# wsakobe/CylinderTag

Measured on AMD Instinct MI355X. Metric: frames/sec detect() 1920x1080, higher is better.
Workload: dtype u8; 1 GPU; synthetic 1920x1080 random-stripe frames, 4096 per step over 1 GPU(s), 4 planted CTag_2f12c markers each, detect(img,5,true,5), inputs resident in HBM; frames_per_gpu=4096, chunk=4096, parallelism=frames sharded, dp1, gather=none (1 GPU)

## Files before the change

### cylindertag_amd/csrc/ctag_internal.h

```cpp
#pragma once
#include <hip/hip_runtime.h>
#include <stddef.h>
#include <stdint.h>

#include <vector>

#include "../../include/ctag_types.h"

struct ctag_handle;
struct ctag_camera;
struct ctag_pose_rec;
struct ctag_rig_pose_rec;
struct ctag_mv_pose_rec;
struct ctag_camera_set;

namespace ctag {
template <class T>
struct DevBuf {
    T* p = nullptr;
    size_t cap = 0;
    DevBuf() = default;
    DevBuf(const DevBuf&) = delete;
    DevBuf& operator=(const DevBuf&) = delete;
    ~DevBuf() { release(); }
// ... 282 lines not shown
    CclForm ccl;
    bool latency;
    bool small_cfg;
    bool refprm;
    bool mask_scan, prescan;
    bool all_wave, fork;
    int pack_max, big_points, pack_gx, scan_gx, mscan_gx, big_cols, big_max_gx, welsch_gs, welsch_gx;
    RefineForm refine; int refine_gx, refine_sums_gx;
    bool ccl_stamps, quad_stamps, feat_stamps;
};
ChunkPlan plan_chunk(const PlanIn& in);

hipError_t launch_zero_counters(const ChunkPlan& pl, const Workspace& ws, hipStream_t s);
hipError_t launch_decimate(const ChunkPlan& pl, const uint8_t* frames, ptrdiff_t frame_stride, ptrdiff_t row_stride, const Workspace& ws, hipStream_t s);
hipError_t launch_threshold_ccl(const ChunkPlan& pl, const Workspace& ws, hipStream_t s);
hipError_t launch_seam_merge(const ChunkPlan& pl, const Workspace& ws, hipStream_t s);
hipError_t launch_resolve(const ChunkPlan& pl, const Workspace& ws, hipStream_t s);
hipError_t launch_candidates(const ChunkPlan& pl, const Workspace& ws, hipStream_t s);
hipError_t launch_quads(const ChunkPlan& pl, const Workspace& ws, hipStream_t s, hipEvent_t* ev5 = nullptr);
hipError_t launch_line_fits(const ChunkPlan& pl, const Workspace& ws, hipStream_t s, unsigned long long* stamps = nullptr, hipEvent_t ev_sorted = nullptr);
int welsch_limits(int32_t* out, int capacity);
hipError_t launch_features(const ChunkPlan& pl, const Workspace& ws, const DetectParams& p, hipStream_t s);
hipError_t launch_edge_refine(const ChunkPlan& pl, const uint8_t* frames, ptrdiff_t frame_stride, ptrdiff_t row_stride, const Workspace& ws, const DetectParams& p, hipStream_t s);
hipError_t launch_markers(const ChunkPlan& pl, const Workspace& ws, const DetectParams& p, ctag_frame_result* out, const PendingCtx& pend, hipStream_t s);
hipError_t launch_counters(int nframes, const Workspace& ws, const ctag_frame_result* results, long long* out10, hipStream_t s);
size_t threshold_ccl_lds_bytes(int tw);
bool build_threshold_table(float dark_cap, uint8_t* table , int* dim, int* tcap);
void build_pick_table(uint8_t* table, uint16_t* table16);


enum SiblingState { kPoseState, kDrawState, kRigState, kGatherState, kMvState, kCovState, kFitState, kRigFitState, kCamFitState, kIntrFitState, kRobustState, kTrackState, kHandEyeState, kNumSiblingStates };
void** handle_state_slot(struct ::ctag_handle* h, SiblingState which, void (*free_fn)(void*));
int model_to_device(struct ::ctag_model* m, int device);
int rigs_to_device(struct ::ctag_rigs* r, int device);
bool camera_ok(const struct ::ctag_camera* c);
bool handle_timing(const struct ::ctag_handle* h);
int handle_finish_pending(struct ::ctag_handle* h);
bool handle_pending_state(struct ::ctag_handle* h, const int32_t** count_dev, uint64_t* gen);
void handle_pending_clean(struct ::ctag_handle* h, uint64_t gen);
int handle_device(const struct ::ctag_handle* h);
int handle_dict_cols(const struct ::ctag_handle* h);

struct HandleView {
    int device;
    const Workspace* ws;
    int last_chunk_frames;
// ... 39 lines not shown
```

### cylindertag_amd/csrc/k_feature.hip

```cpp
#include "ctag_internal.h"
#include "ctag_math.h"
#include "ctag_refine.h"
#include "ctag_wave.h"

namespace ctag {

constexpr double kPi = 3.1415926535897932384626433832795;

struct P2 {
    float x, y;
};
__device__ __forceinline__ float dist2p(P2 a, P2 b) { return ctm::sqrt32((a.x - b.x) * (a.x - b.x) + (a.y - b.y) * (a.y - b.y)); }
__device__ __forceinline__ double angdeg(float dy, float dx) { return ctm::atan2_32(dy, dx) * 180 / kPi; }

struct QuadDerived {
    float cx, cy, d[4], a1, a2;
    float e[4];
};
static_assert(sizeof(QuadDerived) == 48, "workspace carve in ctag_api.hip");
struct FeatPtrs {
    const int32_t* ncand;
    const QuadOut* quads;
    QuadDerived* derived;
    int32_t* quad_index;
// ... 433 lines not shown
    const double* Ll = A + ((it + 1) & 3) * 12 + 6;
    const double A00 = Ln[3], A01 = -Ll[3];
    const double A10 = -Ln[2], A11 = Ll[2];
    const double B0 = -Ln[0] + Ll[0];
    const double B1 = -Ln[1] + Ll[1];
    const double det = A00 * A11 - A10 * A01;
    const double W00 = A11 / det, W01 = -A01 / det;
    const double L0 = W00 * B0 + W01 * B1;
    const int idx = ((it + 1) & 3) + off;
    if (ctm::fabs64(det) > 0.001) {
        O->c[2 * idx] = (float)(Ln[0] + L0 * A00);
        O->c[2 * idx + 1] = (float)(Ln[1] + L0 * A10);
    } else {
        O->c[2 * idx] = F->c[2 * idx];
        O->c[2 * idx + 1] = F->c[2 * idx + 1];
    }
}

#if defined(CTAG_REFINE_PLAIN_SYNC) && CTAG_REFINE_PLAIN_SYNC
__device__ __forceinline__ void refine_sync() { __syncthreads(); }
__device__ __forceinline__ void sums_sync() { __syncthreads(); }
#else
__device__ __forceinline__ void refine_sync() { lds_barrier(); }
__device__ __forceinline__ void sums_sync() { lds_wait(); }
#endif
template <int MODE, int REGION = kRefineRegion>
__device__ __forceinline__ bool refine_quad(const RefinePtrs& P, int rows, int cols, int subpix, int frame, int qidx, int only_long, double alpha128 = 0.0) {
    constexpr int kPitch = kRefineSamples + 1;
    constexpr int kRows = 16;
#ifndef CTAG_ONES_SHIFT
#define CTAG_ONES_SHIFT 16
#endif
    __shared__ __attribute__((aligned(16))) double s_vall[MODE == 1 ? kPitch : (kRows + 1) * kPitch + CTAG_ONES_SHIFT];
    double (*s_v)[kPitch] = reinterpret_cast<double (*)[kPitch]>(s_vall);
    double* const s_ones = MODE == 1 ? s_vall : s_vall + kRows * kPitch + CTAG_ONES_SHIFT;
    double (*s_bx)[kPitch] = s_v, (*s_by)[kPitch] = s_v + (MODE == 1 ? 0 : 4);
    __shared__ double s_nrm[4][2];
    __shared__ uint64_t s_step[4][2];
    __shared__ double s_acc[48];
    __shared__ __attribute__((aligned(16))) uint8_t s_reg[REGION];
    const int fi = qidx >> 1, quad = qidx & 1;
    const int tid = threadIdx.x;
    const FeatureDev* F = P.feat1 + (size_t)frame * CTAG_MAX_FEATURES + fi;
    const uint8_t* __restrict__ img = P.frames + (ptrdiff_t)frame * P.frame_stride;
    const uint32_t rs = (uint32_t)P.row_stride;
    const int off = quad * 4;
    __shared__ float s_cx[4], s_cy[4];
// ... 214 lines not shown
__global__ __launch_bounds__(kRefineThreads) __attribute__((amdgpu_waves_per_eu(MODE == 1 ? (REGION > 36864 ? 3 : CTAG_REFINE_SEARCH_WAVES) : 1, MODE == 1 ? CTAG_REFINE_SEARCH_WAVES : 8)))
void k_edge_refine(RefinePtrs P, int rows, int cols, int subpix, int nframes, int per_frame) {
    int frame = blockIdx.y, bx = blockIdx.x, gx = gridDim.x;
    if (per_frame > 0) {
        const int b = blockIdx.x;
        frame = ((b >> 3) / per_frame) * 8 + (b & 7);
        bx = (b >> 3) % per_frame;
        gx = per_frame;
    }
    if (frame >= nframes) return;
    if (P.status[frame] != CTAG_OK) return;
    const int nq = 2 * min(P.nfeat[frame], CTAG_MAX_FEATURES);
    const double alpha128 = (15.0 + (double)((int)threadIdx.x & (kRefineSamples - 1))) / (kRefineSamples + 30);
    for (int q = bx; q < nq; q += gx) {
        refine_quad<MODE, REGION>(P, rows, cols, subpix, frame, q, 0, alpha128);
        if (q + gx < nq) refine_sync();
    }
}
#ifndef CTAG_REFINE_SUMS2_WAVES
#define CTAG_REFINE_SUMS2_WAVES 4
#endif
constexpr int kSumSeg = 16, kSumSegs = kRefineSamples / kSumSeg;
constexpr int kSumPitch = kSumSeg + 2;
struct SumsPrefetch {
    double n0[kSumSegs];
    float cx, cy;
};
__device__ __forceinline__ void sums_prefetch(const RefinePtrs& P, int frame, int qidx, SumsPrefetch& R) {
    const int tid = threadIdx.x;
    const double* src = P.n0 + ((size_t)frame * (CTAG_MAX_FEATURES * 2) + qidx) * (4 * kRefineSamples) + (tid >> 4) * kRefineSamples + (tid & 15);
#pragma unroll
    for (int g = 0; g < kSumSegs; g++) R.n0[g] = src[g * kSumSeg];
    const FeatureDev* F = P.feat1 + (size_t)frame * CTAG_MAX_FEATURES + (qidx >> 1);
    const int c = (qidx & 1) * 4 + (tid & 3);
    R.cx = F->c[2 * c];
    R.cy = F->c[2 * c + 1];
}
__device__ __forceinline__ bool refine_sums_quad(const SumsPrefetch& pre, const double* s_alpha, double* acc_out) {
    __shared__ __attribute__((aligned(16))) double s_t[48][kSumPitch];
    __shared__ float s_cx[4], s_cy[4];
    __shared__ double s_nrm[4][2];
    __shared__ int s_ns[4];
    const int tid = threadIdx.x;
    if (tid < 4) {
        s_cx[tid] = pre.cx;
        s_cy[tid] = pre.cy;
    }
    sums_sync();
    if (tid < 4) {
        const int a = tid, b = (tid + 1) & 3;
        const double nx = s_cy[b] - s_cy[a];
        const double ny = -s_cx[b] + s_cx[a];
        const double mag = ctm::sqrt64(nx * nx + ny * ny);
        const double ns_d = mag / 8 > 128.0 ? mag / 8 : 128.0;
        s_ns[tid] = (int)ns_d;
        s_nrm[tid][0] = nx / mag;
        s_nrm[tid][1] = ny / mag;
    }
    sums_sync();
    if (max(max(s_ns[0], s_ns[1]), max(s_ns[2], s_ns[3])) > kRefineSamples) return false;
    const int edge = tid >> 4, loc = tid & 15;
    const float ax = s_cx[edge], ay = s_cy[edge], bx = s_cx[(edge + 1) & 3], by = s_cy[(edge + 1) & 3];
    const double nx = s_nrm[edge][0], ny = s_nrm[edge][1];
    double* const mine = &s_t[edge * 12][loc];
    const double2* const row2 = reinterpret_cast<const double2*>(s_t[tid < 48 ? tid : 0]);
    double acc = 0.0;
#pragma unroll
    for (int g = 0; g < kSumSegs; g++) {
        const double alpha = s_alpha[kSumSeg * g + loc];
        const double x0 = alpha * ax + (1 - alpha) * bx;
        const double y0 = alpha * ay + (1 - alpha) * by;
        const double n0 = pre.n0[g];
        const bool ok = n0 == n0;
        const double x = ok ? x0 + n0 * nx : 0.0, y = ok ? y0 + n0 * ny : 0.0;
        const double wn = ok ? 1 - alpha : 0.0, wl = ok ? alpha : 0.0;
        const double xx = x * x, xy = x * y, yy = y * y;
        if (g) sums_sync();
        mine[0 * kSumPitch] = x * wn;
        mine[1 * kSumPitch] = y * wn;
        mine[2 * kSumPitch] = xx * wn;
        mine[3 * kSumPitch] = xy * wn;
        mine[4 * kSumPitch] = yy * wn;
        mine[5 * kSumPitch] = wn;
        mine[6 * kSumPitch] = x * wl;
        mine[7 * kSumPitch] = y * wl;
        mine[8 * kSumPitch] = xx * wl;
        mine[9 * kSumPitch] = xy * wl;
        mine[10 * kSumPitch] = yy * wl;
        mine[11 * kSumPitch] = wl;
        sums_sync();
        if (tid < 48) {
            double t[kSumSeg];
#pragma unroll
            for (int u = 0; u < kSumSeg / 2; u++) {
                const double2 v = row2[u];
                t[2 * u] = v.x, t[2 * u + 1] = v.y;
            }
#pragma unroll
            for (int u = 0; u < kSumSeg; u++) acc += t[u];
        }
    }
    if (tid < 48) acc_out[tid] = acc;
    sums_sync();
    return true;
}
__global__ __launch_bounds__(64) __attribute__((amdgpu_waves_per_eu(CTAG_REFINE_SUMS2_WAVES, 8)))
void k_edge_refine_sums(RefinePtrs P, int nframes, int per_frame) {
    if (blockDim.x != 64) __builtin_trap();
    const int b = blockIdx.x;
    const int frame = ((b >> 3) / per_frame) * 8 + (b & 7);
    const int bx = (b >> 3) % per_frame;
    if (frame >= nframes) return;
    if (P.status[frame] != CTAG_OK) return;
    const int nq = 2 * min(P.nfeat[frame], CTAG_MAX_FEATURES);
    int q = bx;
    if (q >= nq) return;
    __shared__ double s_acc[48];
    __shared__ double s_alpha[kRefineSamples];
    const int tid = threadIdx.x;
    for (int k = tid; k < kRefineSamples; k += 64) s_alpha[k] = (15.0 + k) / (kRefineSamples + 30);
    SumsPrefetch cur, nxt;
    sums_prefetch(P, frame, q, cur);
    vmem_wait();
    int qn = q + per_frame;
    if (qn < nq) sums_prefetch(P, frame, qn, nxt);
    for (;;) {
        const bool have = refine_sums_quad(cur, s_alpha, s_acc);
        const double mine = tid < 48 ? s_acc[tid] : (have ? 1.0 : 0.0);
        double* const out = P.n0 + ((size_t)frame * (CTAG_MAX_FEATURES * 2) + q) * (4 * kRefineSamples);
        sums_sync();
        q = qn;
        qn += per_frame;
        if (q < nq) {
            cur = nxt;
            if (qn < nq) sums_prefetch(P, frame, qn, nxt);
        }
        if (tid < 48 ? have : tid == 48) out[tid] = mine;
        if (q >= nq) break;
    }
}
__global__ __launch_bounds__(64) void k_edge_refine_tail(RefinePtrs P, int nframes, int per_frame) {
    const int frame = blockIdx.y;
    if (frame >= nframes || P.status[frame] != CTAG_OK) return;
    const int nq = 2 * min(P.nfeat[frame], CTAG_MAX_FEATURES);
    __shared__ double s_L[8][48];
    __shared__ int s_ok[8];
    const int tid = threadIdx.x, sl = tid >> 3, ep = tid & 7;
    for (int q0 = (int)blockIdx.x * 8; q0 < nq; q0 += per_frame * 8) {
        const int q = q0 + sl;
        const double* A = P.n0 + ((size_t)frame * (CTAG_MAX_FEATURES * 2) + min(q, nq - 1)) * (4 * kRefineSamples);
        const bool ok = q < nq && A[48] == 1.0;
        if (ep == 0) s_ok[sl] = ok ? 1 : 0;
        if (ok) {
            double a6[6];
#pragma unroll
            for (int k = 0; k < 6; k++) a6[k] = A[(ep >> 1) * 12 + (ep & 1) * 6 + k];
            double* L = s_L[sl] + (ep >> 1) * 12 + (ep & 1) * 6;
            refine_line(a6, L);
        }
        __syncthreads();
        const int sc = tid >> 2;
// ... 668 lines not shown
                out->features[out_features + k] = R;
            }
            out_markers++;
            out_features += rn;
        }
        clk.mark(24);
    }
    if (tid == 0) {
        out->status = CTAG_OK;
        out->n_markers = out_markers;
        out->n_features = out_features;
        out->flags = oflags;
    }
}

static Stamps feat_stamps;

hipError_t launch_features(const ChunkPlan& pl, const Workspace& ws, const DetectParams& p, hipStream_t s) {
    const FeatPtrs P = feat_ptrs(ws, pl.feat_stamps ? feat_stamps.zeroed(s) : nullptr);
    if (pl.latency) hipLaunchKernelGGL(k_features<512>, dim3(pl.nframes), dim3(512), 0, s, P, pl.nframes, p.feature_size);
    else hipLaunchKernelGGL(k_features<128>, dim3(pl.nframes), dim3(128), 0, s, P, pl.nframes, p.feature_size);
    return hipGetLastError();
}
hipError_t launch_edge_refine(const ChunkPlan& pl, const uint8_t* frames, ptrdiff_t frame_stride, ptrdiff_t row_stride, const Workspace& ws, const DetectParams& p, hipStream_t s) {
    const int nframes = pl.nframes, refine_gx = pl.refine_gx, f8 = ((nframes + 7) / 8) * 8;
    const RefinePtrs P = refine_ptrs(frames, frame_stride, row_stride, ws, p);
    if (pl.refine == RefineForm::None) return hipSuccess;
    if (pl.refine == RefineForm::One) {
        hipLaunchKernelGGL(k_edge_refine<0>, dim3(CTAG_MAX_FEATURES * 2, nframes), dim3(kRefineThreads), 0, s, P, ws.g.rows, ws.g.cols, p.subpix_dist, nframes, 0);
        return hipGetLastError();
    }
    if (pl.refine == RefineForm::SplitLarge) hipLaunchKernelGGL((k_edge_refine<1, kRefineRegionLarge>), dim3(f8 * refine_gx), dim3(kRefineThreads), 0, s, P, ws.g.rows, ws.g.cols, p.subpix_dist, nframes, refine_gx);
    else if (pl.refine == RefineForm::SplitLooping) hipLaunchKernelGGL(k_edge_refine<1>, dim3(f8 * refine_gx), dim3(kRefineThreads), 0, s, P, ws.g.rows, ws.g.cols, p.subpix_dist, nframes, refine_gx);
    else hipLaunchKernelGGL(k_edge_refine<1>, dim3(refine_gx, nframes), dim3(kRefineThreads), 0, s, P, ws.g.rows, ws.g.cols, p.subpix_dist, nframes, 0);
    hipLaunchKernelGGL(k_edge_refine_sums, dim3(f8 * pl.refine_sums_gx), dim3(64), 0, s, P, nframes, pl.refine_sums_gx);
    hipLaunchKernelGGL(k_edge_refine_tail, dim3(13, nframes), dim3(64), 0, s, P, nframes, 13);
    hipLaunchKernelGGL(k_edge_refine_long, dim3(4, nframes), dim3(kRefineThreads), 0, s, P, ws.g.rows, ws.g.cols, p.subpix_dist, nframes);
    return hipGetLastError();
}
hipError_t launch_markers(const ChunkPlan& pl, const Workspace& ws, const DetectParams& p, ctag_frame_result* out, const PendingCtx& pend, hipStream_t s) {
    const MarkerPtrs P = marker_ptrs(ws, p, out, pend, pl.feat_stamps ? feat_stamps.d : nullptr);
    if (pl.latency) hipLaunchKernelGGL(k_markers<8>, dim3(pl.nframes), dim3(512), 0, s, P, pl.nframes, p.feature_size, p.dict_rows, p.dict_cols);
    else hipLaunchKernelGGL(k_markers<1>, dim3(pl.nframes), dim3(64), 0, s, P, pl.nframes, p.feature_size, p.dict_rows, p.dict_cols);
    if (pl.feat_stamps) {
        unsigned long long h[25];
        feat_stamps.read(s, h, 25);
        fprintf(stderr, "[k_features ticks] compact %llu derive %llu pairs %llu greedy %llu organise %llu obtain %llu\n", h[0], h[1], h[2], h[3], h[4], h[5]);
        fprintf(stderr, "[k_markers ticks] load %llu pairs %llu union %llu sort %llu ids %llu carry+pre %llu | code %llu coverage %llu pick+store %llu\n", h[16], h[17], h[18],
                h[19], h[20], h[21], h[22], h[23], h[24]);
    }
    return hipGetLastError();
}

}
```

### include/ctag_testkit.h

```cpp
#ifndef CTAG_TESTKIT_H
#define CTAG_TESTKIT_H
#include <stddef.h>
#include <stdint.h>

#include "ctag.h"
#include "ctag_pose.h"

#ifdef __cplusplus
extern "C" {
#endif

#define CTAG_DBG_HALF 1
#define CTAG_DBG_LABELS 2
#define CTAG_DBG_CANDIDATES 3
#define CTAG_DBG_CAND_QUADS 4
#define CTAG_DBG_FEATURES0 5
#define CTAG_DBG_FEATURES1 6
#define CTAG_DBG_FEATURES2 7
#define CTAG_DBG_PREMARKERS 8
#define CTAG_DBG_GRAY 9
#define CTAG_DBG_MASK 11
#define CTAG_DBG_LINES 10
#define CTAG_DBG_LINE_POINTS 12
#define CTAG_DBG_LINE_FITS 13
// ... 61 lines not shown
typedef struct ctag_synth3d_truth {
    int32_t n_markers;
    int32_t dict_row[8];
    double R[8][9];
    double t[8][3];
    double radius[8];
} ctag_synth3d_truth;
int ctag_synth3d_frames_device(ctag_handle* h, uint8_t* frames_dev, int first_frame, int n, int rows, int cols, ptrdiff_t row_stride,
                               ptrdiff_t frame_stride, uint64_t seed, int markers_per_frame, double fx, double fy, double cx, double cy);
int ctag_synth3d_frame_host(const int32_t* state, int dict_rows, int dict_cols, uint8_t* frame, int frame_index, int rows, int cols,
                            ptrdiff_t row_stride, uint64_t seed, int markers_per_frame, double fx, double fy, double cx, double cy,
                            ctag_synth3d_truth* truth);
int ctag_synth3d_model(const int32_t* state, int dict_rows, int dict_cols, float* corners);

int ctag_testkit_dense_edge_probe(ctag_handle* h, const uint8_t* gray, int rows, int cols, ptrdiff_t row_stride, const double* segments,
                                  int n_seg, const double* K, const double* dist, const double* rvec, const double* tvec,
                                  int samples_per_edge, double search_px, double min_contrast, double* out, int32_t* keep);

int ctag_testkit_welsch_fit(ctag_handle* h, int n_frames, const int32_t* edges_per_frame, const int32_t* points_per_edge, const int32_t* xy,
                            int latency, int welsch_gx, int welsch_gs, int tail_at_pool_end, float* lines);

int ctag_testkit_welsch_limits(int32_t* out, int capacity);

int ctag_testkit_model_fit_system(ctag_handle* h, const ctag_frame_result* results, int n_frames, const ctag_pose_rec* poses, int n_poses,
                                  const ctag_model* model, const ctag_camera* camera, int model_index, double lambda, int min_obs, int pass_records,
                                  double* S, double* g, double* delta, int32_t* held, int32_t* bad_pivot);
int ctag_testkit_model_fit_limits(int32_t* out, int capacity);

int ctag_testkit_rig_fit_system(ctag_handle* h, const ctag_frame_result* results, int n_frames, const ctag_rig_pose_rec* rig_poses,
                                const ctag_model* model, const ctag_rigs* rigs, const ctag_camera* camera, int rig, double lambda, int pass_records,
                                double* S, double* g, double* delta, int32_t* n_unknowns, int32_t* bad_pivot);
int ctag_testkit_rig_fit_limits(int32_t* out, int capacity);

int ctag_testkit_camera_fit_system(ctag_handle* h, const ctag_frame_result* results, int n_frames, const ctag_mv_pose_rec* mv_poses,
                                   const ctag_model* model, const ctag_rigs* rigs, const ctag_camera_set* cams, int anchor, double lambda,
                                   int pass_records, double* S, double* g, double* delta, int32_t* n_unknowns, int32_t* bad_pivot);
int ctag_testkit_camera_fit_limits(int32_t* out, int capacity);

int ctag_testkit_intrinsics_fit_system(ctag_handle* h, const ctag_frame_result* results, int n_frames, const ctag_rig_pose_rec* poses,
                                       const ctag_model* model, const ctag_rigs* rigs, const ctag_camera* camera, uint32_t free_mask, int tie_focal,
                                       double lambda, int pass_records, double* S, double* g, double* delta, int32_t* n_free, int32_t* bad_pivot);
int ctag_testkit_intrinsics_fit_poses(ctag_handle* h, const ctag_frame_result* results, int n_frames, const ctag_rig_pose_rec* poses,
                                      const ctag_model* model, const ctag_rigs* rigs, const ctag_camera* camera, ctag_rig_pose_rec* out, int32_t* usable);
int ctag_testkit_intrinsics_fit_limits(int32_t* out, int capacity);

int ctag_testkit_plan(int rows, int cols, int adaptive_thresh, int nframes, int channels, int corner_subpix, const void* frames,
// ... 8 lines not shown
```

### testkit/__init__.py

```python
import ctypes as C
import os
import subprocess

import numpy as np

import cylindertag_amd as ca
from cylindertag_amd import capi
from cylindertag_amd.capi import CtagError, Model

_HERE = os.path.dirname(os.path.abspath(__file__))
_LIB = os.environ.get("CTAG_TESTKIT_LIB") or os.path.join(_HERE, "_build", "libctag_testkit.so")

TRUTH3D_DT = np.dtype([("n_markers", "<i4"), ("dict_row", "<i4", (8,)), ("_pad", "<i4", (1,)), ("R", "<f8", (8, 9)), ("t", "<f8", (8, 3)),
                       ("radius", "<f8", (8,))])
TRUTH_DT = np.dtype([("n_markers", "<i4"), ("dict_row", "<i4", (8,)), ("strip_len", "<f4", (8,)),
                     ("corners", "<f4", (8, 8))])
DBG_HALF, DBG_LABELS, DBG_CANDIDATES, DBG_CAND_QUADS, DBG_FEATURES0, DBG_FEATURES1, DBG_FEATURES2, DBG_PREMARKERS, DBG_GRAY, DBG_LINES, DBG_MASK, DBG_LINE_POINTS, DBG_LINE_FITS, DBG_PACKS, DBG_PACKS1 = range(1, 16)
SYNTH_SEED = 0x4354616753594E00

EXPORTS = ["ctag_debug_fetch", "ctag_math_probe", "ctag_testkit_wave_probe", "ctag_testkit_exp32_k0_sweep", "ctag_testkit_unpack_gathered", "ctag_testkit_stall_stream", "ctag_synth_frames_device", "ctag_synth_frame_host",
           "ctag_synth_layout_truth", "ctag_synth3d_frames_device", "ctag_synth3d_frame_host", "ctag_synth3d_model",
           "ctag_testkit_dense_edge_probe", "ctag_testkit_plan", "ctag_testkit_welsch_fit", "ctag_testkit_welsch_limits",
           "ctag_testkit_model_fit_system", "ctag_testkit_model_fit_limits", "ctag_testkit_rig_fit_system", "ctag_testkit_rig_fit_limits",
           "ctag_testkit_camera_fit_system", "ctag_testkit_camera_fit_limits",
           "ctag_testkit_intrinsics_fit_system", "ctag_testkit_intrinsics_fit_poses", "ctag_testkit_intrinsics_fit_limits"]
PLAN_FIELDS = ("fused", "bgr_direct", "zero_first", "dec_zero_kernel", "dec_zero_list", "dec", "dec_xblocks", "dec_yblocks", "dec_band_rows", "dec_bands",
               "ccl", "latency", "small_cfg", "refprm", "mask_scan", "prescan", "all_wave", "fork", "pack_max", "big_points", "pack_gx", "scan_gx",
               "mscan_gx", "big_cols", "big_max_gx", "welsch_gs", "welsch_gx", "refine", "refine_gx", "refine_sums_gx")
DEC_FORMS = ("mask", "mask_bands", "general", "wide", "banded135", "banded", "unaligned")
CCL_FORMS = ("mask", "tw5", "any")
WELSCH_LIMITS = ("kWShort", "kWCap", "kWRes", "kWPts", "kWPtsU", "kPickN", "kPickN2", "kWE", "kWT", "kLatLines", "kLatPoints", "kLatChunk", "kLdsLines",
                 "kLatencyFrames", "kLatRankBlocks", "kLineSortBuckets")
REFINE_FORMS = ("none", "one", "split_large", "split_looping", "split")
MATH_EXP32_NONPOS, MATH_EXP32_NONPOS_K0, MATH_LOG64 = 15, 17, 18
WAVE_OPS = ("FROM_PREV", "FROM_NEXT", "SHR1_I32", "SHR2_I32", "SHR4_I32", "SHR1_F32", "SHR1_F64", "XOR1_I32", "XOR2_I32", "HALF_MIRROR_I32", "ROW_MIRROR_I32",
            "XOR1_I64", "XOR2_I64", "HALF_MIRROR_I64", "ROW_MIRROR_I64", "INCL_SCAN", "SG_SUM8_I32", "SG_SUM64_I32", "SG_SUM8_I64", "SG_SUM64_I64",
            "SG_BEST8_NEAREST", "SG_BEST8_FARTHEST", "SG_BEST64_NEAREST", "SG_BEST64_FARTHEST", "SUM_F64", "MAX_F64", "ALL", "PK_MIN_U16", "PK_MAX_U16")
for _i, _n in enumerate(WAVE_OPS):
    globals()["WAVE_" + _n] = _i
WAVE_SENTINEL_F64, WAVE_SENTINEL_I64 = -12345.6789, -0x5a5a5a5a5a5a5a5a


def lib_path():
    return _LIB

# ... 31 lines not shown
    L.ctag_synth_frames_device.argtypes = [vp, vp, C.c_int, C.c_int, C.c_int, C.c_int, C.c_ssize_t, C.c_ssize_t,
                                           C.c_uint64, C.c_int]
    L.ctag_synth_frame_host.restype = C.c_int
    L.ctag_synth_frame_host.argtypes = [i32p, C.c_int, C.c_int, vp, C.c_int, C.c_int, C.c_int, C.c_ssize_t, C.c_uint64,
                                        C.c_int, vp]
    L.ctag_synth_layout_truth.restype = C.c_int
    L.ctag_synth_layout_truth.argtypes = [i32p, C.c_int, C.c_int, C.c_int, C.c_int, C.c_int, C.c_uint64, C.c_int, vp]
    L.ctag_synth3d_frames_device.restype = C.c_int
    L.ctag_synth3d_frames_device.argtypes = [vp, vp, C.c_int, C.c_int, C.c_int, C.c_int, C.c_ssize_t, C.c_ssize_t, C.c_uint64, C.c_int,
                                             C.c_double, C.c_double, C.c_double, C.c_double]
    L.ctag_synth3d_frame_host.restype = C.c_int
    L.ctag_synth3d_frame_host.argtypes = [i32p, C.c_int, C.c_int, vp, C.c_int, C.c_int, C.c_int, C.c_ssize_t, C.c_uint64, C.c_int, C.c_double,
                                          C.c_double, C.c_double, C.c_double, vp]
    L.ctag_synth3d_model.restype = C.c_int
    L.ctag_synth3d_model.argtypes = [i32p, C.c_int, C.c_int, vp]
    L.ctag_testkit_plan.restype = C.c_int
    L.ctag_testkit_plan.argtypes = [C.c_int, C.c_int, C.c_int, C.c_int, C.c_int, C.c_int, vp, C.c_ssize_t, C.c_ssize_t, C.c_int, C.c_int, C.c_int,
                                    C.c_int, i32p, C.c_int]
    L.ctag_testkit_dense_edge_probe.restype = C.c_int
    L.ctag_testkit_dense_edge_probe.argtypes = [vp, vp, C.c_int, C.c_int, C.c_ssize_t, vp, C.c_int, vp, vp, vp, vp, C.c_int,
                                                C.c_double, C.c_double, vp, vp]
    L.ctag_testkit_welsch_fit.restype = C.c_int
    L.ctag_testkit_welsch_fit.argtypes = [vp, C.c_int, vp, vp, vp, C.c_int, C.c_int, C.c_int, C.c_int, vp]
    L.ctag_testkit_welsch_limits.restype = C.c_int
    L.ctag_testkit_welsch_limits.argtypes = [i32p, C.c_int]
    L.ctag_testkit_model_fit_system.restype = C.c_int
    L.ctag_testkit_model_fit_system.argtypes = [vp, vp, C.c_int, vp, C.c_int, vp, C.POINTER(capi.CameraC), C.c_int, C.c_double, C.c_int, C.c_int, vp, vp, vp,
                                                vp, i32p]
    L.ctag_testkit_model_fit_limits.restype = C.c_int
    L.ctag_testkit_model_fit_limits.argtypes = [i32p, C.c_int]
    L.ctag_testkit_rig_fit_system.restype = C.c_int
    L.ctag_testkit_rig_fit_system.argtypes = [vp, vp, C.c_int, vp, vp, vp, C.POINTER(capi.CameraC), C.c_int, C.c_double, C.c_int, vp, vp, vp, i32p, i32p]
    L.ctag_testkit_rig_fit_limits.restype = C.c_int
    L.ctag_testkit_rig_fit_limits.argtypes = [i32p, C.c_int]
    L.ctag_testkit_camera_fit_system.restype = C.c_int
    L.ctag_testkit_camera_fit_system.argtypes = [vp, vp, C.c_int, vp, vp, vp, vp, C.c_int, C.c_double, C.c_int, vp, vp, vp, i32p, i32p]
    L.ctag_testkit_camera_fit_limits.restype = C.c_int
    L.ctag_testkit_camera_fit_limits.argtypes = [i32p, C.c_int]
    L.ctag_testkit_intrinsics_fit_system.restype = C.c_int
    L.ctag_testkit_intrinsics_fit_system.argtypes = [vp, vp, C.c_int, vp, vp, vp, C.POINTER(capi.CameraC), C.c_uint32, C.c_int, C.c_double, C.c_int, vp, vp, vp,
                                                     i32p, i32p]
    L.ctag_testkit_intrinsics_fit_poses.restype = C.c_int
    L.ctag_testkit_intrinsics_fit_poses.argtypes = [vp, vp, C.c_int, vp, vp, vp, C.POINTER(capi.CameraC), vp, i32p]
    L.ctag_testkit_intrinsics_fit_limits.restype = C.c_int
    L.ctag_testkit_intrinsics_fit_limits.argtypes = [i32p, C.c_int]
    _lib = L
# ... 160 lines not shown
            return a.reshape(-1, 8)
        if what in (DBG_FEATURES0, DBG_FEATURES1, DBG_FEATURES2):
            return a.reshape(-1, 19)
        if what == DBG_PREMARKERS:
            return a[0]
        if what == DBG_LINE_POINTS:
            return a.reshape(-1, 2)
        if what == DBG_LINE_FITS:
            return a.reshape(-1, 4)
        return a

    def welsch_fit(self, frames, latency=0, welsch_gx=0, welsch_gs=0, tail_at_pool_end=False):
        clusters = [np.asarray(c, np.int32).reshape(-1, 2) for f in frames for c in f]
        edges = np.array([len(f) for f in frames], np.int32)
        counts = np.array([len(c) for c in clusters], np.int32)
        xy = np.ascontiguousarray(np.concatenate(clusters) if clusters else np.zeros((0, 2)), np.int32)
        lines = np.zeros((len(clusters), 4), np.float32)
        st = self.T.ctag_testkit_welsch_fit(self.h, len(frames), edges.ctypes.data, counts.ctypes.data, xy.ctypes.data, int(latency), int(welsch_gx),
                                            int(welsch_gs), int(bool(tail_at_pool_end)), lines.ctypes.data)
        if st != 0:
            raise CtagError(st, "ctag_testkit_welsch_fit")
        return lines

    def model_fit_system(self, results, poses, model, camera, model_index, lam, min_obs=2, pass_records=0):
        res = np.ascontiguousarray(results).reshape(-1)
        assert res.dtype == ca.RESULT_DT
        poses = np.ascontiguousarray(poses, ca.POSE_DT).reshape(-1)
        P = int(model.view()["size"]) * 8
        S, g, d = np.zeros((3 * P, 3 * P)), np.zeros(3 * P), np.zeros(3 * P)
        held = np.zeros(P, np.int32)
        bad = C.c_int32()
        st = self.T.ctag_testkit_model_fit_system(self.h, res.ctypes.data, len(res), poses.ctypes.data, len(poses), model.m, C.byref(camera),
                                                  int(model_index), float(lam), int(min_obs), int(pass_records), S.ctypes.data, g.ctypes.data,
                                                  d.ctypes.data, held.ctypes.data, C.byref(bad))
        if st != 0:
            raise CtagError(st, "ctag_testkit_model_fit_system")
        return {"S": S, "g": g, "delta": d, "held": held.astype(bool), "bad_pivot": bool(bad.value)}

    def rig_fit_system(self, results, rig_poses, model, rigs, camera, rig, lam, pass_records=0):
        res = np.ascontiguousarray(results).reshape(-1)
        assert res.dtype == ca.RESULT_DT
        recs = np.ascontiguousarray(rig_poses, ca.RIG_POSE_DT).reshape(-1)
        assert len(recs) == len(res) * rigs.n_rigs
        S, g, d = np.zeros(96 * 96), np.zeros(96), np.zeros(96)
        n, bad = C.c_int32(), C.c_int32()
        st = self.T.ctag_testkit_rig_fit_system(self.h, res.ctypes.data, len(res), recs.ctypes.data, model.m, rigs.r, C.byref(camera), int(rig),
# ... 88 lines not shown
```

### testkit/ctag_testkit.hip

```cpp
#include <hip/hip_runtime.h>

#include <algorithm>
#include <cstring>
#include <vector>

#include "../include/ctag_testkit.h"
#include "../cylindertag_amd/csrc/ctag_internal.h"
#include "../cylindertag_amd/csrc/ctag_math.h"
#include "../cylindertag_amd/csrc/ctag_wave.h"
#include "ctag_synth.h"

using namespace ctag;

#define TK_TRY(expr)                              \
    do {                                          \
        if ((expr) != hipSuccess) return CTAG_ERR_HIP; \
    } while (0)

namespace {

__global__ void k_math_probe(int op, int n, const double* a, const double* b, double* out) {
    const int i = blockIdx.x * blockDim.x + threadIdx.x;
    if (i >= n) return;
    const double x = a[i], y = b[i];
// ... 762 lines not shown
        TK_TRY(hipMemsetAsync(W.line_fit + (size_t)f * W.line_cap * 4, 0xff, desc[f].size() * 16, s));
    }
    const FrameGeom& g = W.g;
    ChunkPlan pl = plan_chunk(PlanIn{g.rows, g.cols, g.tw, n_frames, 1, 1, nullptr, 0, 0, W.kp, 0, 0, false, DevKnobs{}});
    pl.latency = latency != 0;
    if (welsch_gx > 0) pl.welsch_gx = welsch_gx;
    if (welsch_gs > 0) pl.welsch_gs = welsch_gs;
    if (launch_line_fits(pl, W, s) != hipSuccess) {
        (void)hipGetLastError();
        return CTAG_ERR_HIP;
    }
    TK_TRY(hipStreamSynchronize(s));
    e0 = 0;
    for (int f = 0; f < n_frames; f++) {
        if (desc[f].empty()) continue;
        TK_TRY(hipMemcpy(lines + e0 * 4, W.line_fit + (size_t)f * W.line_cap * 4, desc[f].size() * 16, hipMemcpyDeviceToHost));
        e0 += desc[f].size();
    }
    return CTAG_OK;
}

int ctag_testkit_welsch_limits(int32_t* out, int capacity) { return welsch_limits(out, out ? std::max(capacity, 0) : 0); }

int ctag_testkit_model_fit_system(ctag_handle* h, const ctag_frame_result* results, int n_frames, const ctag_pose_rec* poses, int n_poses,
                                  const ctag_model* model, const ctag_camera* camera, int model_index, double lambda, int min_obs, int pass_records,
                                  double* S, double* g, double* delta, int32_t* held, int32_t* bad_pivot) {
    return mfit_probe_system(h, results, n_frames, poses, n_poses, model, camera, model_index, lambda, min_obs, pass_records, S, g, delta, held, bad_pivot);
}

int ctag_testkit_model_fit_limits(int32_t* out, int capacity) {
    const int32_t v[2] = {mfit_record_grid(), mfit_pass_records()};
    if (out) std::memcpy(out, v, sizeof(int32_t) * (size_t)std::min(std::max(capacity, 0), 2));
    return 2;
}

int ctag_testkit_rig_fit_system(ctag_handle* h, const ctag_frame_result* results, int n_frames, const ctag_rig_pose_rec* rig_poses,
                                const ctag_model* model, const ctag_rigs* rigs, const ctag_camera* camera, int rig, double lambda, int pass_records,
                                double* S, double* g, double* delta, int32_t* n_unknowns, int32_t* bad_pivot) {
    return rfit_probe_system(h, results, n_frames, rig_poses, model, rigs, camera, rig, lambda, pass_records, S, g, delta, n_unknowns, bad_pivot);
}

int ctag_testkit_rig_fit_limits(int32_t* out, int capacity) {
    const int32_t v[2] = {rfit_record_grid(), rfit_pass_records()};
    if (out) std::memcpy(out, v, sizeof(int32_t) * (size_t)std::min(std::max(capacity, 0), 2));
    return 2;
}
// ... 50 lines not shown
```

Measured before the change: 289,000 frames/s.

## Process two quads per block in refine-sums with constant-memory weights

Restructures k_edge_refine_sums so each 64-thread block handles two quads per iteration, storing 6 unweighted moment rows per edge in LDS. The (1-alpha)/alpha weighting moves into the reduction through a constant-memory weight table, which halves the LDS stores and barriers per quad. It also prefetches the next pair's n0 values and corners inside the loop, tightens sums_sync with an explicit waitcnt, and adds a testkit entry point for checking the kernel on its own. The risks are higher register pressure from the doubled prefetch arrays and the weight loads, plus small numerical differences because weights are now applied after summation.

```diff
diff --git a/cylindertag_amd/csrc/ctag_internal.h b/cylindertag_amd/csrc/ctag_internal.h
--- a/cylindertag_amd/csrc/ctag_internal.h
+++ b/cylindertag_amd/csrc/ctag_internal.h
@@ -328,6 +328,7 @@
 int welsch_limits(int32_t* out, int capacity);
 hipError_t launch_features(const ChunkPlan& pl, const Workspace& ws, const DetectParams& p, hipStream_t s);
 hipError_t launch_edge_refine(const ChunkPlan& pl, const uint8_t* frames, ptrdiff_t frame_stride, ptrdiff_t row_stride, const Workspace& ws, const DetectParams& p, hipStream_t s);
+hipError_t launch_edge_refine_sums(const ChunkPlan& pl, const Workspace& ws, hipStream_t s);
 hipError_t launch_markers(const ChunkPlan& pl, const Workspace& ws, const DetectParams& p, ctag_frame_result* out, const PendingCtx& pend, hipStream_t s);
 hipError_t launch_counters(int nframes, const Workspace& ws, const ctag_frame_result* results, long long* out10, hipStream_t s);
 size_t threshold_ccl_lds_bytes(int tw);
diff --git a/cylindertag_amd/csrc/k_feature.hip b/cylindertag_amd/csrc/k_feature.hip
--- a/cylindertag_amd/csrc/k_feature.hip
+++ b/cylindertag_amd/csrc/k_feature.hip
@@ -479,7 +479,7 @@
 __device__ __forceinline__ void sums_sync() { __syncthreads(); }
 #else
 __device__ __forceinline__ void refine_sync() { lds_barrier(); }
-__device__ __forceinline__ void sums_sync() { lds_wait(); }
+__device__ __forceinline__ void sums_sync() { lds_wait(), __builtin_amdgcn_s_waitcnt(0xc07f); }
 #endif
 template <int MODE, int REGION = kRefineRegion>
 __device__ __forceinline__ bool refine_quad(const RefinePtrs& P, int rows, int cols, int subpix, int frame, int qidx, int only_long, double alpha128 = 0.0) {
@@ -740,88 +740,23 @@
 #endif
 constexpr int kSumSeg = 16, kSumSegs = kRefineSamples / kSumSeg;
 constexpr int kSumPitch = kSumSeg + 2;
+constexpr int kSumRows = 24;
+struct SumsWeights {
+    double w[kRefineSamples][2];
+    constexpr SumsWeights() : w{} {
+        for (int s = 0; s < kRefineSamples; s++) {
+            const double alpha = (15.0 + s) / (kRefineSamples + 30);
+            w[s][0] = 1 - alpha;
+            w[s][1] = alpha;
+        }
+    }
+};
+__constant__ SumsWeights c_sums_w = SumsWeights();
+typedef const double __attribute__((address_space(4))) * SumsWeightPtr;
 struct SumsPrefetch {
-    double n0[kSumSegs];
+    double n0[2][kSumSegs];
     float cx, cy;
 };
-__device__ __forceinline__ void sums_prefetch(const RefinePtrs& P, int frame, int qidx, SumsPrefetch& R) {
-    const int tid = threadIdx.x;
-    const double* src = P.n0 + ((size_t)frame * (CTAG_MAX_FEATURES * 2) + qidx) * (4 * kRefineSamples) + (tid >> 4) * kRefineSamples + (tid & 15);
-#pragma unroll
-    for (int g = 0; g < kSumSegs; g++) R.n0[g] = src[g * kSumSeg];
-    const FeatureDev* F = P.feat1 + (size_t)frame * CTAG_MAX_FEATURES + (qidx >> 1);
-    const int c = (qidx & 1) * 4 + (tid & 3);
-    R.cx = F->c[2 * c];
-    R.cy = F->c[2 * c + 1];
-}
-__device__ __forceinline__ bool refine_sums_quad(const SumsPrefetch& pre, const double* s_alpha, double* acc_out) {
-    __shared__ __attribute__((aligned(16))) double s_t[48][kSumPitch];
-    __shared__ float s_cx[4], s_cy[4];
-    __shared__ double s_nrm[4][2];
-    __shared__ int s_ns[4];
-    const int tid = threadIdx.x;
-    if (tid < 4) {
-        s_cx[tid] = pre.cx;
-        s_cy[tid] = pre.cy;
-    }
-    sums_sync();
-    if (tid < 4) {
-        const int a = tid, b = (tid + 1) & 3;
-        const double nx = s_cy[b] - s_cy[a];
-        const double ny = -s_cx[b] + s_cx[a];
-        const double mag = ctm::sqrt64(nx * nx + ny * ny);
-        const double ns_d = mag / 8 > 128.0 ? mag / 8 : 128.0;
-        s_ns[tid] = (int)ns_d;
-        s_nrm[tid][0] = nx / mag;
-        s_nrm[tid][1] = ny / mag;
-    }
-    sums_sync();
-    if (max(max(s_ns[0], s_ns[1]), max(s_ns[2], s_ns[3])) > kRefineSamples) return false;
-    const int edge = tid >> 4, loc = tid & 15;
-    const float ax = s_cx[edge], ay = s_cy[edge], bx = s_cx[(edge + 1) & 3], by = s_cy[(edge + 1) & 3];
-    const double nx = s_nrm[edge][0], ny = s_nrm[edge][1];
-    double* const mine = &s_t[edge * 12][loc];
-    const double2* const row2 = reinterpret_cast<const double2*>(s_t[tid < 48 ? tid : 0]);
-    double acc = 0.0;
-#pragma unroll
-    for (int g = 0; g < kSumSegs; g++) {
-        const double alpha = s_alpha[kSumSeg * g + loc];
-        const double x0 = alpha * ax + (1 - alpha) * bx;
-        const double y0 = alpha * ay + (1 - alpha) * by;
-        const double n0 = pre.n0[g];
-        const bool ok = n0 == n0;
-        const double x = ok ? x0 + n0 * nx : 0.0, y = ok ? y0 + n0 * ny : 0.0;
-        const double wn = ok ? 1 - alpha : 0.0, wl = ok ? alpha : 0.0;
-        const double xx = x * x, xy = x * y, yy = y * y;
-        if (g) sums_sync();
-        mine[0 * kSumPitch] = x * wn;
-        mine[1 * kSumPitch] = y * wn;
-        mine[2 * kSumPitch] = xx * wn;
-        mine[3 * kSumPitch] = xy * wn;
-        mine[4 * kSumPitch] = yy * wn;
-        mine[5 * kSumPitch] = wn;
-        mine[6 * kSumPitch] = x * wl;
-        mine[7 * kSumPitch] = y * wl;
-        mine[8 * kSumPitch] = xx * wl;
-        mine[9 * kSumPitch] = xy * wl;
-        mine[10 * kSumPitch] = yy * wl;
-        mine[11 * kSumPitch] = wl;
-        sums_sync();
-        if (tid < 48) {
-            double t[kSumSeg];
-#pragma unroll
-            for (int u = 0; u < kSumSeg / 2; u++) {
-                const double2 v = row2[u];
-                t[2 * u] = v.x, t[2 * u + 1] = v.y;
-            }
-#pragma unroll
-            for (int u = 0; u < kSumSeg; u++) acc += t[u];
-        }
-    }
-    if (tid < 48) acc_out[tid] = acc;
-    sums_sync();
-    return true;
-}
 __global__ __launch_bounds__(64) __attribute__((amdgpu_waves_per_eu(CTAG_REFINE_SUMS2_WAVES, 8)))
 void k_edge_refine_sums(RefinePtrs P, int nframes, int per_frame) {
     if (blockDim.x != 64) __builtin_trap();
@@ -831,30 +766,133 @@
     if (frame >= nframes) return;
     if (P.status[frame] != CTAG_OK) return;
     const int nq = 2 * min(P.nfeat[frame], CTAG_MAX_FEATURES);
-    int q = bx;
-    if (q >= nq) return;
-    __shared__ double s_acc[48];
+    if (bx >= nq) return;
+    __shared__ __attribute__((aligned(16))) double s_t[2 * kSumRows][kSumPitch];
+    __shared__ float s_cx[8], s_cy[8];
+    __shared__ double s_nrm[8][2];
+    __shared__ int s_ns[8];
     __shared__ double s_alpha[kRefineSamples];
     const int tid = threadIdx.x;
     for (int k = tid; k < kRefineSamples; k += 64) s_alpha[k] = (15.0 + k) / (kRefineSamples + 30);
-    SumsPrefetch cur, nxt;
-    sums_prefetch(P, frame, q, cur);
+    const int edge = tid >> 4, loc = tid & 15;
+    double* const n0_frame = P.n0 + (size_t)frame * (CTAG_MAX_FEATURES * 2) * (4 * kRefineSamples);
+    const uint32_t lane_off = (uint32_t)((edge * kRefineSamples + loc) * sizeof(double));
+    constexpr uint32_t kSegBytes = kSumSeg * sizeof(double);
+    auto n0_at = [](const double* base, uint32_t off) -> double { return *reinterpret_cast<const double*>(reinterpret_cast<const char*>(base) + off); };
+    const FeatureDev* const F_frame = P.feat1 + (size_t)frame * CTAG_MAX_FEATURES;
+    SumsPrefetch pre;
+    auto request_corner = [&](int qa, int qb) {
+        const int qi = (tid & 4) ? qb : qa;
+        const FeatureDev* F = F_frame + (qi >> 1);
+        const int c = (qi & 1) * 4 + (tid & 3);
+        pre.cx = F->c[2 * c];
+        pre.cy = F->c[2 * c + 1];
+    };
+    int q0 = bx, q1 = bx + per_frame;
+    const int step = 2 * per_frame;
+    request_corner(q0, q1 < nq ? q1 : q0);
+#pragma unroll
+    for (int g = 0; g < kSumSegs; g++) {
+        pre.n0[0][g] = n0_at(n0_frame + (size_t)q0 * (4 * kRefineSamples), lane_off + g * kSegBytes);
+        pre.n0[1][g] = 0.0;
+        if (q1 < nq) pre.n0[1][g] = n0_at(n0_frame + (size_t)q1 * (4 * kRefineSamples), lane_off + g * kSegBytes);
+    }
     vmem_wait();
-    int qn = q + per_frame;
-    if (qn < nq) sums_prefetch(P, frame, qn, nxt);
+    sums_sync();
+    const double2* const row2 = reinterpret_cast<const double2*>(s_t[tid < 2 * kSumRows ? tid : 0]);
     for (;;) {
-        const bool have = refine_sums_quad(cur, s_alpha, s_acc);
-        const double mine = tid < 48 ? s_acc[tid] : (have ? 1.0 : 0.0);
-        double* const out = P.n0 + ((size_t)frame * (CTAG_MAX_FEATURES * 2) + q) * (4 * kRefineSamples);
+        const bool have1 = q1 < nq;
+        const int nq0 = q0 + step, nq1 = q1 + step;
+        const bool next0 = nq0 < nq, next1 = nq1 < nq;
+        if (tid < 8) {
+            s_cx[tid] = pre.cx;
+            s_cy[tid] = pre.cy;
+        }
         sums_sync();
-        q = qn;
-        qn += per_frame;
-        if (q < nq) {
-            cur = nxt;
-            if (qn < nq) sums_prefetch(P, frame, qn, nxt);
-        }
-        if (tid < 48 ? have : tid == 48) out[tid] = mine;
-        if (q >= nq) break;
+        request_corner(next0 ? nq0 : q0, next1 ? nq1 : q0);
+        if (tid < 8) {
+            const int a = tid, b = (tid & 4) | ((tid + 1) & 3);
+            const double nx = s_cy[b] - s_cy[a];
+            const double ny = -s_cx[b] + s_cx[a];
+            const double mag = ctm::sqrt64(nx * nx + ny * ny);
+            const double ns_d = mag / 8 > 128.0 ? mag / 8 : 128.0;
+            s_ns[tid] = (int)ns_d;
+            s_nrm[tid][0] = nx / mag;
+            s_nrm[tid][1] = ny / mag;
+        }
+        sums_sync();
+        const bool do0 = __builtin_amdgcn_readfirstlane(max(max(s_ns[0], s_ns[1]), max(s_ns[2], s_ns[3]))) <= kRefineSamples;
+        const bool do1 = have1 && __builtin_amdgcn_readfirstlane(max(max(s_ns[4], s_ns[5]), max(s_ns[6], s_ns[7]))) <= kRefineSamples;
+        float ax[2], ay[2], bx_[2], by[2];
+        double nx[2], ny[2];
+#pragma unroll
+        for (int sl = 0; sl < 2; sl++) {
+            ax[sl] = s_cx[4 * sl + edge], ay[sl] = s_cy[4 * sl + edge], bx_[sl] = s_cx[4 * sl + ((edge + 1) & 3)], by[sl] = s_cy[4 * sl + ((edge + 1) & 3)];
+            nx[sl] = s_nrm[4 * sl + edge][0], ny[sl] = s_nrm[4 * sl + edge][1];
+        }
+        const double* const nbase[2] = {n0_frame + (size_t)(next0 ? nq0 : 0) * (4 * kRefineSamples), n0_frame + (size_t)(next1 ? nq1 : 0) * (4 * kRefineSamples)};
+        const uint32_t noff[2] = {next0 ? lane_off : 0u, next1 ? lane_off : 0u};
+        double accN = 0.0, accL = 0.0;
+        double alpha_next = s_alpha[loc];
+#pragma unroll
+        for (int g = 0; g < kSumSegs; g++) {
+            const double alpha = alpha_next;
+            if (g) sums_sync();
+            SumsWeightPtr wp = (SumsWeightPtr)&c_sums_w.w[kSumSeg * g][0];
+            asm volatile("" : "+s"(wp));
+            double w[2 * kSumSeg];
+#pragma unroll
+            for (int u = 0; u < 2 * kSumSeg; u++) w[u] = wp[u];
+#pragma unroll
+            for (int sl = 0; sl < 2; sl++) {
+                const double x0 = alpha * ax[sl] + (1 - alpha) * bx_[sl];
+                const double y0 = alpha * ay[sl] + (1 - alpha) * by[sl];
+                const double n0 = pre.n0[sl][g];
+                const bool ok = n0 == n0;
+                const double x = ok ? x0 + n0 * nx[sl] : 0.0, y = ok ? y0 + n0 * ny[sl] : 0.0;
+                double* const mine = &s_t[sl * kSumRows + edge * 6][loc];
+                mine[0 * kSumPitch] = x;
+                mine[1 * kSumPitch] = y;
+                mine[2 * kSumPitch] = x * x;
+                mine[3 * kSumPitch] = x * y;
+                mine[4 * kSumPitch] = y * y;
+                mine[5 * kSumPitch] = ok ? 1.0 : 0.0;
+                pre.n0[sl][g] = n0_at(nbase[sl], noff[sl] + ((sl ? next1 : next0) ? g * kSegBytes : 0u));
+            }
+            if (g + 1 < kSumSegs) alpha_next = s_alpha[kSumSeg * (g + 1) + loc];
+            sums_sync();
+            if (tid < 2 * kSumRows) {
+                double t[kSumSeg];
+#pragma unroll
+                for (int u = 0; u < kSumSeg / 2; u++) {
+                    const double2 v = row2[u];
+                    t[2 * u] = v.x, t[2 * u + 1] = v.y;
+                }
+#pragma unroll
+                for (int u = 0; u < kSumSeg; u++) {
+                    accN += t[u] * w[2 * u];
+                    accL += t[u] * w[2 * u + 1];
+                }
+            }
+        }
+        {
+            const int sl = tid >= kSumRows ? 1 : 0, r = tid - sl * kSumRows;
+            const int e = r / 6, m = r - e * 6;
+            double* const out = n0_frame + (size_t)(sl ? q1 : q0) * (4 * kRefineSamples);
+            if (tid < 2 * kSumRows) {
+                if (sl ? do1 : do0) {
+                    out[e * 12 + m] = accN;
+                    out[e * 12 + 6 + m] = accL;
+                }
+            } else if (tid == 48) {
+                n0_frame[(size_t)q0 * (4 * kRefineSamples) + 48] = do0 ? 1.0 : 0.0;
+            } else if (tid == 49 && have1) {
+                n0_frame[(size_t)q1 * (4 * kRefineSamples) + 48] = do1 ? 1.0 : 0.0;
+            }
+        }
+        if (!next0) break;
+        q0 = nq0, q1 = nq1;
+        sums_sync();
     }
 }
 __global__ __launch_bounds__(64) void k_edge_refine_tail(RefinePtrs P, int nframes, int per_frame) {
@@ -1569,6 +1607,14 @@
     else hipLaunchKernelGGL(k_features<128>, dim3(pl.nframes), dim3(128), 0, s, P, pl.nframes, p.feature_size);
     return hipGetLastError();
 }
+static void launch_refine_sums(const ChunkPlan& pl, const RefinePtrs& P, hipStream_t s) {
+    const int f8 = ((pl.nframes + 7) / 8) * 8;
+    hipLaunchKernelGGL(k_edge_refine_sums, dim3(f8 * pl.refine_sums_gx), dim3(64), 0, s, P, pl.nframes, pl.refine_sums_gx);
+}
+hipError_t launch_edge_refine_sums(const ChunkPlan& pl, const Workspace& ws, hipStream_t s) {
+    launch_refine_sums(pl, refine_ptrs(nullptr, 0, 0, ws, DetectParams{}), s);
+    return hipGetLastError();
+}
 hipError_t launch_edge_refine(const ChunkPlan& pl, const uint8_t* frames, ptrdiff_t frame_stride, ptrdiff_t row_stride, const Workspace& ws, const DetectParams& p, hipStream_t s) {
     const int nframes = pl.nframes, refine_gx = pl.refine_gx, f8 = ((nframes + 7) / 8) * 8;
     const RefinePtrs P = refine_ptrs(frames, frame_stride, row_stride, ws, p);
@@ -1580,7 +1626,7 @@
     if (pl.refine == RefineForm::SplitLarge) hipLaunchKernelGGL((k_edge_refine<1, kRefineRegionLarge>), dim3(f8 * refine_gx), dim3(kRefineThreads), 0, s, P, ws.g.rows, ws.g.cols, p.subpix_dist, nframes, refine_gx);
     else if (pl.refine == RefineForm::SplitLooping) hipLaunchKernelGGL(k_edge_refine<1>, dim3(f8 * refine_gx), dim3(kRefineThreads), 0, s, P, ws.g.rows, ws.g.cols, p.subpix_dist, nframes, refine_gx);
     else hipLaunchKernelGGL(k_edge_refine<1>, dim3(refine_gx, nframes), dim3(kRefineThreads), 0, s, P, ws.g.rows, ws.g.cols, p.subpix_dist, nframes, 0);
-    hipLaunchKernelGGL(k_edge_refine_sums, dim3(f8 * pl.refine_sums_gx), dim3(64), 0, s, P, nframes, pl.refine_sums_gx);
+    launch_refine_sums(pl, P, s);
     hipLaunchKernelGGL(k_edge_refine_tail, dim3(13, nframes), dim3(64), 0, s, P, nframes, 13);
     hipLaunchKernelGGL(k_edge_refine_long, dim3(4, nframes), dim3(kRefineThreads), 0, s, P, ws.g.rows, ws.g.cols, p.subpix_dist, nframes);
     return hipGetLastError();
diff --git a/include/ctag_testkit.h b/include/ctag_testkit.h
--- a/include/ctag_testkit.h
+++ b/include/ctag_testkit.h
@@ -107,6 +107,9 @@
 
 int ctag_testkit_welsch_limits(int32_t* out, int capacity);
 
+int ctag_testkit_refine_sums(ctag_handle* h, int n_frames, const int32_t* nfeat, const int32_t* status, const float* corners, const double* n0,
+                             double* sums);
+
 int ctag_testkit_model_fit_system(ctag_handle* h, const ctag_frame_result* results, int n_frames, const ctag_pose_rec* poses, int n_poses,
                                   const ctag_model* model, const ctag_camera* camera, int model_index, double lambda, int min_obs, int pass_records,
                                   double* S, double* g, double* delta, int32_t* held, int32_t* bad_pivot);
diff --git a/testkit/__init__.py b/testkit/__init__.py
--- a/testkit/__init__.py
+++ b/testkit/__init__.py
@@ -20,7 +20,7 @@
 
 EXPORTS = ["ctag_debug_fetch", "ctag_math_probe", "ctag_testkit_wave_probe", "ctag_testkit_exp32_k0_sweep", "ctag_testkit_unpack_gathered", "ctag_testkit_stall_stream", "ctag_synth_frames_device", "ctag_synth_frame_host",
            "ctag_synth_layout_truth", "ctag_synth3d_frames_device", "ctag_synth3d_frame_host", "ctag_synth3d_model",
-           "ctag_testkit_dense_edge_probe", "ctag_testkit_plan", "ctag_testkit_welsch_fit", "ctag_testkit_welsch_limits",
+           "ctag_testkit_dense_edge_probe", "ctag_testkit_plan", "ctag_testkit_welsch_fit", "ctag_testkit_welsch_limits", "ctag_testkit_refine_sums",
            "ctag_testkit_model_fit_system", "ctag_testkit_model_fit_limits", "ctag_testkit_rig_fit_system", "ctag_testkit_rig_fit_limits",
            "ctag_testkit_camera_fit_system", "ctag_testkit_camera_fit_limits",
            "ctag_testkit_intrinsics_fit_system", "ctag_testkit_intrinsics_fit_poses", "ctag_testkit_intrinsics_fit_limits"]
@@ -98,6 +98,8 @@
                                                 C.c_double, C.c_double, vp, vp]
     L.ctag_testkit_welsch_fit.restype = C.c_int
     L.ctag_testkit_welsch_fit.argtypes = [vp, C.c_int, vp, vp, vp, C.c_int, C.c_int, C.c_int, C.c_int, vp]
+    L.ctag_testkit_refine_sums.restype = C.c_int
+    L.ctag_testkit_refine_sums.argtypes = [vp, C.c_int, vp, vp, vp, vp, vp]
     L.ctag_testkit_welsch_limits.restype = C.c_int
     L.ctag_testkit_welsch_limits.argtypes = [i32p, C.c_int]
     L.ctag_testkit_model_fit_system.restype = C.c_int
@@ -304,6 +306,18 @@
             raise CtagError(st, "ctag_testkit_welsch_fit")
         return lines
 
+    def refine_sums(self, nfeat, status, corners, n0):
+        nfeat = np.ascontiguousarray(nfeat, np.int32)
+        status = np.ascontiguousarray(status, np.int32)
+        nq = 2 * int(nfeat.sum())
+        corners = np.ascontiguousarray(corners, np.float32).reshape(nq // 2, 16)
+        n0 = np.ascontiguousarray(n0, np.float64).reshape(nq, 4, 128)
+        sums = np.zeros((nq, 49), np.float64)
+        st = self.T.ctag_testkit_refine_sums(self.h, len(nfeat), nfeat.ctypes.data, status.ctypes.data, corners.ctypes.data, n0.ctypes.data, sums.ctypes.data)
+        if st != 0:
+            raise CtagError(st, "ctag_testkit_refine_sums")
+        return sums
+
     def model_fit_system(self, results, poses, model, camera, model_index, lam, min_obs=2, pass_records=0):
         res = np.ascontiguousarray(results).reshape(-1)
         assert res.dtype == ca.RESULT_DT
diff --git a/testkit/ctag_testkit.hip b/testkit/ctag_testkit.hip
--- a/testkit/ctag_testkit.hip
+++ b/testkit/ctag_testkit.hip
@@ -808,6 +808,56 @@
 
 int ctag_testkit_welsch_limits(int32_t* out, int capacity) { return welsch_limits(out, out ? std::max(capacity, 0) : 0); }
 
+int ctag_testkit_refine_sums(ctag_handle* h, int n_frames, const int32_t* nfeat, const int32_t* status, const float* corners, const double* n0, double* sums) {
+    if (!h || n_frames < 1 || !nfeat || !status) return CTAG_ERR_ARG;
+    HandleView v{};
+    handle_view(h, &v);
+    if (!v.ws || !v.ws->base || !v.ws->refine_n0 || n_frames > v.last_chunk_frames) return CTAG_ERR_ARG;
+    const Workspace& W = *v.ws;
+    size_t total = 0;
+    for (int f = 0; f < n_frames; f++) {
+        if (nfeat[f] < 0 || nfeat[f] > CTAG_MAX_FEATURES) return CTAG_ERR_ARG;
+        total += (size_t)nfeat[f];
+    }
+    if (total > 0 && (!corners || !n0 || !sums)) return CTAG_ERR_ARG;
+    const FrameGeom& g = W.g;
+    const ChunkPlan pl = plan_chunk(PlanIn{g.rows, g.cols, g.tw, n_frames, 1, 1, nullptr, 0, 0, W.kp, 0, 0, false, DevKnobs{}});
+    if (pl.refine == RefineForm::None || pl.refine == RefineForm::One) return CTAG_ERR_ARG;
+    constexpr size_t kQuad = 4 * 128;
+    TK_TRY(hipSetDevice(v.device));
+    hipStream_t s = static_cast<hipStream_t>(ctag_stream(h));
+    TK_TRY(hipStreamSynchronize(s));
+    TK_TRY(hipMemcpy(W.nfeat, nfeat, (size_t)n_frames * 4, hipMemcpyHostToDevice));
+    TK_TRY(hipMemcpy(W.status, status, (size_t)n_frames * 4, hipMemcpyHostToDevice));
+    size_t f0 = 0;
+    for (int f = 0; f < n_frames; f++) {
+        const size_t nf = (size_t)nfeat[f];
+        if (nf == 0) continue;
+        std::vector<FeatureDev> feats(nf);
+        for (size_t k = 0; k < nf; k++) {
+            FeatureDev F{};
+            std::memcpy(F.c, corners + (f0 + k) * 16, sizeof(F.c));
+            feats[k] = F;
+        }
+        TK_TRY(hipMemcpy(W.feat1 + (size_t)f * CTAG_MAX_FEATURES, feats.data(), nf * sizeof(FeatureDev), hipMemcpyHostToDevice));
+        TK_TRY(hipMemcpy(W.refine_n0 + (size_t)f * (CTAG_MAX_FEATURES * 2) * kQuad, n0 + f0 * 2 * kQuad, nf * 2 * kQuad * 8, hipMemcpyHostToDevice));
+        f0 += nf;
+    }
+    if (launch_edge_refine_sums(pl, W, s) != hipSuccess) {
+        (void)hipGetLastError();
+        return CTAG_ERR_HIP;
+    }
+    TK_TRY(hipStreamSynchronize(s));
+    f0 = 0;
+    for (int f = 0; f < n_frames; f++) {
+        const size_t nq = (size_t)nfeat[f] * 2;
+        if (nq == 0) continue;
+        TK_TRY(hipMemcpy2D(sums + f0 * 49, 49 * 8, W.refine_n0 + (size_t)f * (CTAG_MAX_FEATURES * 2) * kQuad, kQuad * 8, 49 * 8, nq, hipMemcpyDeviceToHost));
+        f0 += nq;
+    }
+    return CTAG_OK;
+}
+
 int ctag_testkit_model_fit_system(ctag_handle* h, const ctag_frame_result* results, int n_frames, const ctag_pose_rec* poses, int n_poses,
                                   const ctag_model* model, const ctag_camera* camera, int model_index, double lambda, int min_obs, int pass_records,
                                   double* S, double* g, double* delta, int32_t* held, int32_t* bad_pivot) {
```

Measured after the change: 293,100 frames/s (median of 6 runs). +1.4%, better.
